# BenjSta/bernoulli-var-speech-codec

Measured on AMD Instinct MI355X. Metric: audio-seconds coded per wall-second (encode+decode), 22.05 kHz @ 3 kbit/s, higher is better.
Workload: dtype f32; 1 GPU; BASELINE configs[1]: batch 64 x 5 s utterances per GPU, config_varBitRate @ 3000 bit/s (35 bits/frame), full encode -> BigVGAN decode; one batch at a time on one stream; frames_per_utterance=430, weights=seeded synthetic (checkpoints are LFS pointers), gather=none, streams=1

## Files before the change

bernoulli-var-speech-codec_amd/csrc/bvc_internal.h:

```cpp
#pragma once
#include <hip/hip_runtime.h>
#include <stdint.h>
#include <string>
#include <vector>

#include "../../include/bvcodec.h"

namespace bvc {

void set_error(const char *fmt, ...);

#define BVC_HIP_TRY(expr)                                                              \
    do {                                                                               \
        hipError_t e_ = (expr);                                                        \
        if (e_ != hipSuccess) {                                                        \
            bvc::set_error("%s failed: %s (%s:%d)", #expr, hipGetErrorString(e_), __FILE__, __LINE__); \
            return BVC_EHIP;                                                           \
        }                                                                              \
    } while (0)

enum ProbeKind { PK_NONE = 0, PK_LINEAR = 1, PK_GRU = 2, PK_CONV = 3, PK_BATCHED = 4, PK_STFT = 5, PK_POST = 6 };
struct ProbeScope {
    hipStream_t s; int slot;
    ProbeScope(int kind, hipStream_t stream);
// ... 101 lines not shown
    int wnb;
    int pad_;
};
struct FlowArgs {
    FlowLin enc0h, enc1, enc2, pz0, pz1, pz2, dec0h, dec0z, dec1, dec2, dec3, px0, px1, px2;
    const float *w_hh, *w_ihx, *w_ihz;
    const float *b_ih, *b_hh;
    int hb, zb, xb;
    float *flow; unsigned slot_bytes;
    int B, MT, NTG;
    long long T;
    const float *part0;
    const float *part_gru;
    float *codes, *prob; const float *bits; float *all_h; float *mel;
    const float *mean, *stdv;
    int var_bit;
    unsigned *status; unsigned spin_limit;
    unsigned long long *probe;
    int probe_nodes, probe_first;
    int probe_wg, probe_wave;
    int dbg_hot_w;
    int MG;
    int dbg_withhold;
    FlowLin pxc;
    float *keep;
};
int flow_kernels_init();
int flow_perh(int h_dim);
int launch_flow(const FlowArgs &a, FlowArgs *d_args, int perh, bool encode, bool fill, hipStream_t s, bool args_resident = false);
int launch_flow_prepare(const FlowArgs &a, FlowArgs *d_args, unsigned *flow, long long n_flow, long long n_h0, const float *d_h0, int B, int H,
                        hipStream_t s);
int launch_flow_census(unsigned *ctr, int grid, unsigned spin_limit, hipStream_t s);
int launch_fill_u32(unsigned *p, unsigned v, long long n, hipStream_t s);

struct FrontendTables {
    const float *window;
    const float2 *tw1;
    const float2 *tw2;
    const float2 *tws;
    const int   *mel_start;
    const int   *mel_len;
    const int   *mel_off;
    const float *mel_w;
    int num_mels;
    int kmax;
};
int launch_stft_logmel(const FrontendTables &t, const float *wav, int B, long long L, long long T,
                       int pad_left, float scale, float *mel, hipStream_t s, const long long *lens = nullptr);
__host__ __device__ inline long long ragged_frames(long long len, long long L, int pad_left) {
    len = len < 0 ? 0 : (len > L ? L : len);
    const long long pr = 1024 - 256 - pad_left;
    if (len <= pad_left || len <= pr) return 0;
    return (len + pad_left + pr - 1024) / 256 + 1;
}
int launch_ragged_bits(float *bits, const float *d_bits, float dflt, const long long *lens, int B, long long L, long long T,
                       int pad_left, hipStream_t s);
int launch_ragged_mask(float *codes, const long long *lens, int B, long long L, long long T, int z, int pad_left, hipStream_t s);

int launch_resample_poly(const float *x, int B, long long Lin, const double *h, int ntaps, int up, int down,
                         long long n_pre_remove, float *y, long long n_out, hipStream_t s);
int launch_peak_normalize(float *x, int B, long long L, hipStream_t s);
int launch_pack_codes(const float *codes, long long frames, int z, int nbits, unsigned char *out, hipStream_t s);
int launch_unpack_codes(const unsigned char *in, long long frames, int z, int nbits, float *codes, hipStream_t s);

struct ConvLayer {
    int cin;
    int cout;
    int ntiles;
    int ks;
    int dil;
    const float *wp;
    const float *wp4;
    const float *wp2;
    const float *bias;
    const float *act_a;
    const float *act_ib;
};
enum ConvEpi { CE_STORE = 0, CE_RES = 1, CE_RES_ACC = 2, CE_RES_ACC_DIV = 3 };
#ifdef BVC_PHASE_PROBE
int phase_probe_read(unsigned long long *out, int reset);
#endif
struct ConvWindow { long long in_bs, out_bs, row_begin, t_origin; };
int conv_kernels_init();
enum : unsigned { AMPK_C8 = 1u, AMPK_C16 = 2u, AMPK_ALL = 3u };
unsigned amp_kernels_default();
int launch_snakebeta_test(const float *x, long long n, float a, float ib, float *y, hipStream_t s);
int launch_conv_mfma(const ConvLayer &c, const float *in, long long Lin, float *out, long long Lout,
                     int B, int epi, const float *res, const float *acc, float divisor, hipStream_t s,
                     const ConvWindow *win = nullptr, const long long *row_lim = nullptr);
int launch_amp_pair(const ConvLayer &c1, const ConvLayer &c2, const float *x, long long L, float *out, int B, int epi,
                    const float *acc, float divisor, hipStream_t s, const ConvWindow *win = nullptr, unsigned kernels = AMPK_ALL);
int launch_conv_post(const float *in, long long Lin, int C, int ks, const float *w, const float *bias,
                     const float *act_a, const float *act_ib, float div, float *wav, long long n_out,
                     int B, hipStream_t s, const ConvWindow *win = nullptr, const long long *n_rows = nullptr);
int launch_ragged_limits(long long *lim, const long long *frames, const long long *lengths, int B, long long T, long long n_max,
                         int n_up, const int *up_rates, hipStream_t s);

}
```

bernoulli-var-speech-codec_amd/csrc/bvcodec_abi.hip:

```cpp
#include <algorithm>
#include <atomic>
#include <cmath>
#include <cstdarg>
#include <cstdio>
#include <cstdlib>
#include <cstring>
#include <list>
#include <map>
#include <memory>
#include <mutex>

#include "bvc_internal.h"

namespace bvc {

static thread_local char g_err[512] = "";

void set_error(const char *fmt, ...) {
    va_list ap;
    va_start(ap, fmt);
    vsnprintf(g_err, sizeof(g_err), fmt, ap);
    va_end(ap);
}

// ... 1963 lines not shown
    hipStream_t s = (hipStream_t)stream;
    const int B = st->B;
    sc_append_kernel<<<dim3((unsigned)((st->hop + 255) / 256), B), 256, 0, s>>>(st->d_state, st->d_in, st->hop, st->sbuf, st->cap);
    if (st->first) {
        sc_reflect_left_kernel<<<dim3(B), 256, 0, s>>>(st->sbuf, st->cap, c.pad_left);
        st->first = false;
    }
    BVC_HIP_TRY(hipGetLastError());
    const int fill = st->fill + st->hop;
    const int k = fill >= c.n_fft ? (fill - c.n_fft) / c.hop + 1 : 0;
    if (k > st->kmax) { set_error("bvc_stream_codec_tick: internal frame count %d", k); return BVC_EINVAL; }
    int rc = BVC_OK;
    if (k > 0) {
        const int parity = st->voc->parity;
        const bool tick_flow = st->tick_flow && flow_chains_static(st->m, B) != 0;
        const bool warm = !tick_flow && !st->voc->slide && st->use_graph && s != nullptr && st->frames >= STREAM_WARM_FRAMES;
        g_stream_tick = true; g_tick_flow = tick_flow;
        if (!warm) {
            rc = stream_tick_body(st, k, s);
        } else {
            hipGraphExec_t &ge = st->graph[k][parity];
            if (!ge) {
                hipGraph_t graph = nullptr;
                const int vp = st->voc->parity; const int64_t vf = st->voc->frames;
                g_capturing = true;
                hipError_t e = hipStreamBeginCapture(s, hipStreamCaptureModeThreadLocal);
                if (e == hipSuccess) rc = stream_tick_body(st, k, s);
                hipError_t e2 = (e == hipSuccess) ? hipStreamEndCapture(s, &graph) : e;
                g_capturing = false;
                st->voc->parity = vp; st->voc->frames = vf;
                if (!rc && (e2 != hipSuccess || !graph)) { set_error("bvc_stream_codec_tick: hipGraph capture failed: %s", hipGetErrorString(e2)); rc = BVC_EHIP; }
                if (!rc && hipGraphInstantiate(&ge, graph, nullptr, nullptr, 0) != hipSuccess) { set_error("bvc_stream_codec_tick: hipGraphInstantiate failed"); rc = BVC_EHIP; }
                if (graph) (void)hipGraphDestroy(graph);
            }
            if (!rc) {
                if (hipGraphLaunch(ge, s) != hipSuccess) { set_error("bvc_stream_codec_tick: hipGraphLaunch failed"); rc = BVC_EHIP; }
                st->voc->parity ^= 1; st->voc->frames += k;
            }
        }
        g_stream_tick = false; g_tick_flow = false;
        if (rc) return rc;
    }
    sc_advance_kernel<<<1, 64, 0, s>>>(st->d_state, st->hop - c.hop * k);
    BVC_HIP_TRY(hipGetLastError());
    st->fill = fill - c.hop * k;
    st->frames += k;
    st->ticks += 1;
    if (n_frames) *n_frames = k;
    return BVC_OK;
}

int bvc_model_set_option(bvc_model *m, const char *name, int32_t value) {
    if (!m || !name) { set_error("bvc_model_set_option: null argument"); return BVC_EINVAL; }
    if (strcmp(name, "recurrence") == 0) {
        if (value < 0 || value > 2) { set_error("bvc_model_set_option: recurrence must be 0 (persistent), 1 (layers) or 2 (auto)"); return BVC_EINVAL; }
        m->recurrence = value;
        return BVC_OK;
    }
    if (strcmp(name, "flow_spin_limit") == 0) {
        if (value < 1) { set_error("bvc_model_set_option: flow_spin_limit must be positive"); return BVC_EINVAL; }
        m->flow_spin_limit = (unsigned)value;
        return BVC_OK;
    }
    if (strcmp(name, "flow_debug_withhold") == 0) {
        m->flow_debug_withhold = value != 0;
        return BVC_OK;
    }
    if (strcmp(name, "decode_fold") == 0) {
        m->decode_fold = value != 0;
        return BVC_OK;
    }
    if (strcmp(name, "encode_fold") == 0) {
        m->encode_fold = value != 0;
        return BVC_OK;
    }
    if (strcmp(name, "flow_debug_nofill") == 0) {
        m->flow_debug_nofill = value != 0;
        return BVC_OK;
    }
    if (strcmp(name, "vocoder_c16_kernel") == 0) {
        m->amp_kernels = value ? (m->amp_kernels | AMPK_C16) : (m->amp_kernels & ~AMPK_C16);
        return BVC_OK;
    }
    if (strcmp(name, "vocoder_full_tiles") == 0) {
        m->amp_kernels = value ? (m->amp_kernels | AMPK_C8) : (m->amp_kernels & ~AMPK_C8);
        return BVC_OK;
    }
    set_error("bvc_model_set_option: unknown option '%s'", name);
    return BVC_EINVAL;
}

int bvc_flow_fence(void *stream) {
    hipStream_t s = (hipStream_t)stream;
    hipStreamCaptureStatus cs = hipStreamCaptureStatusNone;
    BVC_HIP_TRY(hipStreamIsCapturing(s, &cs));
    if (cs != hipStreamCaptureStatusNone) { set_error("bvc_flow_fence: not while the stream is being captured"); return BVC_EINVAL; }
    int dev = 0;
    BVC_HIP_TRY(hipGetDevice(&dev));
    dev &= 15;
    std::lock_guard<std::mutex> lk(g_flow_mu);
    FlowFence &f = g_fence[dev][g_fence_n[dev]++ % FLOW_FENCES];
    if (!f.ev) BVC_HIP_TRY(hipEventCreateWithFlags(&f.ev, hipEventDisableTiming));
    if (f.pending) BVC_HIP_TRY(hipStreamWaitEvent(s, f.ev, 0));
    BVC_HIP_TRY(hipEventRecord(f.ev, s));
    f.pending = true;
    return BVC_OK;
}

int bvc_model_get_option(const bvc_model *m, const char *name, int32_t *value) {
    if (!m || !name || !value) { set_error("bvc_model_get_option: null argument"); return BVC_EINVAL; }
    if (strcmp(name, "recurrence") == 0) { *value = m->recurrence; return BVC_OK; }
    if (strcmp(name, "decode_fold") == 0) { *value = m->decode_fold; return BVC_OK; }
    if (strcmp(name, "encode_fold") == 0) { *value = m->encode_fold; return BVC_OK; }
    if (strcmp(name, "flow_resident") == 0) { *value = m->flow_resident ? 1 : 0; return BVC_OK; }
    if (strcmp(name, "flow_supported") == 0) { *value = m->flow_perh > 0 ? 1 : 0; return BVC_OK; }
    if (strcmp(name, "compute_units") == 0) { *value = m->cu_count; return BVC_OK; }
    set_error("bvc_model_get_option: unknown option '%s'", name);
    return BVC_EINVAL;
}

int bvc_model_status(const bvc_model *m, uint32_t *code) {
    if (!m) { set_error("null model"); return BVC_EINVAL; }
    unsigned v = 0;
    if (m->h_status) {
        BVC_HIP_TRY(hipDeviceSynchronize());
        v = *m->h_status;
        if (v) { *m->h_status = 0u; m->census_due = true; }
    }
    if (code) *code = v;
    if (v) {
        set_error("a persistent recurrence kernel gave up waiting (frame %u, layer %u): its results are invalid",
                  (v & 0x7FFFFFFFu) >> 4, (v & 15u));
        return BVC_ETIMEOUT;
    }
    return BVC_OK;
}

int bvc_model_poll_status(const bvc_model *m, uint32_t *code) {
    if (!m) { set_error("null model"); return BVC_EINVAL; }
    unsigned v = 0;
    if (m->h_status) {
        v = *m->h_status;
        if (v) { *m->h_status = 0u; m->census_due = true; }
    }
    if (code) *code = v;
    if (v) {
        set_error("a persistent recurrence kernel gave up waiting (frame %u, layer %u): the results of the call that has just been "
                  "synchronised are invalid.  All its workgroups must be resident together - is another process using this GPU?",
                  (v & 0x7FFFFFFFu) >> 4, (v & 15u));
        return BVC_ETIMEOUT;
    }
    return BVC_OK;
}

int bvc_probe_begin(int32_t kind, int32_t sample_every, int32_t max_samples) {
    if (kind <= PK_NONE || kind > PK_POST || sample_every < 1 || max_samples < 1) {
        set_error("bvc_probe_begin: bad arguments");
        return BVC_EINVAL;
    }
    while ((int)g_probe.ev.size() < 2 * max_samples) {
        hipEvent_t e;
        BVC_HIP_TRY(hipEventCreate(&e));
        g_probe.ev.push_back(e);
    }
    g_probe.kind = kind; g_probe.every = sample_every; g_probe.counter = 0; g_probe.used = 0;
    return BVC_OK;
// ... 159 lines not shown
```

bernoulli-var-speech-codec_amd/csrc/k_vocoder.hip:

```cpp
#include <cstdlib>
#include <type_traits>

#include "bvc_internal.h"

namespace bvc {

typedef float f32x4 __attribute__((ext_vector_type(4)));

__device__ __forceinline__ void divide_if(bool div, f32x4 &v, float d) {
    if (div) {
        asm volatile("" ::: "memory");
#pragma unroll
        for (int e = 0; e < 4; ++e) v[e] = v[e] / d;
    }
}

__device__ __forceinline__ unsigned div_tpb(unsigned bid, unsigned tpb_magic) { return __umulhi(bid, tpb_magic); }
static inline unsigned tpb_magic_of(unsigned d) { return d <= 1u ? 0xFFFFFFFFu : (unsigned)(0x100000000ull / d) + 1u; }

__device__ __forceinline__ __amdgpu_buffer_rsrc_t rows_rsrc(const float *base, long long L, int C) {
    return __builtin_amdgcn_make_buffer_rsrc(const_cast<float *>(base), 0, (int)(L * C * 4), 0x00020000);
}
__device__ __forceinline__ f32x4 rows_load4(__amdgpu_buffer_rsrc_t rs, int row, int C, int c0) {
    return __builtin_bit_cast(f32x4, __builtin_amdgcn_raw_buffer_load_b128(rs, (row * C + c0) * 4, 0, 0));
// ... 367 lines not shown
            const float hi1 = __int_as_float(__builtin_amdgcn_update_dpp(0, __float_as_int(a3), 0x118, 0xf, 0xf, false));
            const float v0 = r < 8 ? a0 : hi0, v1 = r < 8 ? a1 : hi1;
            const int row = mbase + i * 16 + g * 4 + e0;
            const f32x2 s2 = snakebeta2((f32x2){v0 + bias, v1 + bias}, splat2(aa), splat2(bb));
            t2[row * S + col] = row >= zrow ? s2[0] : 0.0f;
            t2[(row + 1) * S + col] = row + 1 >= zrow ? s2[1] : 0.0f;
        }
    } else {
        auto s2_tile = [&](auto edge_c) {
            constexpr bool EDGE = decltype(edge_c)::value;
#pragma unroll
            for (int n = 0; n < NTL; ++n) {
                const int col = (nt0 + n) * 16 + r;
                if (col < C) {
                    const float bias = a.b1[col], aa = a.a2[col], bb = a.ib2[col];
#pragma unroll
                    for (int i = 0; i < MT; ++i)
#pragma unroll
                        for (int e = 0; e < 4; e += 2) {
                            const int row = mbase + i * 16 + g * 4 + e;
                            const f32x2 u2 = (f32x2){acc[i][n][e] + bias, acc[i][n][e + 1] + bias};
                            const f32x2 s2 = snakebeta2(u2, splat2(aa), splat2(bb));
                            t2[row * S + col] = (!EDGE || row >= zrow) ? s2[0] : 0.0f;
                            t2[(row + 1) * S + col] = (!EDGE || row + 1 >= zrow) ? s2[1] : 0.0f;
                        }
                }
            }
        };
        if (zrow > 0) s2_tile(std::true_type());
        else          s2_tile(std::false_type());
    }
    __syncthreads();
    PHASE(2);

    const long long ob = (long long)b * a.bs + t0 * C;
    constexpr int NLD3 = (TR * C4 + 255) / 256;
    const long long rows_left = a.L - t0;
    const int nvalid4 = (int)(rows_left < TT ? rows_left : TT) * C4;
    f32x4 resq[NLD3], accq[NLD3];
    const bool with_acc = a.epi >= CE_RES_ACC;
#pragma unroll
    for (int i = 0; i < NLD3; ++i) {
        const int idx = tid + i * 256;
        const int idc = idx < nvalid4 ? idx : 0;
        resq[i] = reinterpret_cast<const f32x4 *>(a.x + ob)[idc];
        accq[i] = with_acc ? reinterpret_cast<const f32x4 *>(a.acc + ob)[idc] : (f32x4){0.f, 0.f, 0.f, 0.f};
    }
    PHASE(3);
    conv(t2, 1, a.w2);
    PHASE(4);
    if (ALIAS) __syncthreads();
#pragma unroll
    for (int n = 0; n < NTL; ++n) {
        const int col = (nt0 + n) * 16 + r;
        if (col >= C) continue;
        const float bias = a.b2[col];
#pragma unroll
        for (int i = 0; i < MT; ++i)
#pragma unroll
            for (int e = 0; e < 4; ++e) t1[(mbase + i * 16 + g * 4 + e) * S + col] = acc[i][n][e] + bias;
    }
    __syncthreads();
#pragma unroll
    for (int i = 0; i < NLD3; ++i) {
        const int idx = tid + i * 256;
        if (idx >= nvalid4) continue;
        const int row = idx / C4, c4 = idx - row * C4;
        const float2 lo = *reinterpret_cast<const float2 *>(t1 + row * S + c4 * 4);
        const float2 hi = *reinterpret_cast<const float2 *>(t1 + row * S + c4 * 4 + 2);
        f32x4 v = (f32x4){lo.x, lo.y, hi.x, hi.y};
#pragma unroll
        for (int e = 0; e < 4; ++e) {
            float o = v[e] + resq[i][e];
            if (a.epi >= CE_RES_ACC) o = accq[i][e] + o;
            v[e] = o;
        }
        divide_if(a.epi == CE_RES_ACC_DIV, v, a.divisor);
        reinterpret_cast<f32x4 *>(a.out + ob)[idx] = v;
    }
    PHASE(5);
}

unsigned amp_kernels_default() {
    return (getenv("BVC_NO_AMP8") == nullptr ? AMPK_C8 : 0u) | (getenv("BVC_NO_AMP16") == nullptr ? AMPK_C16 : 0u);
}

template <int D>
__device__ __forceinline__ int pair_row(int m) { return (m / D) * (2 * D) + m % D; }
template <int D>
__device__ __forceinline__ int row_pos(int rho, int H) {
    const int blk = rho / (2 * D), w = rho - blk * (2 * D);
    return w >= D ? H + blk * D + (w - D) : blk * D + w;
}
template <int KS, int D, int MT2>
struct Amp8Geom {
    static constexpr int NP = 4 * MT2 * 16;
    static constexpr int NPE = (NP / D) * D;
    static constexpr int TR1 = 2 * NPE;
    static constexpr int TR = 2 * NP;
    static constexpr int TT = TR1 - (KS - 1);
    static constexpr int HALO1 = (KS - 1) * D;
    static constexpr int ROWS1 = TR1 + HALO1;
    static constexpr int H1 = NP + ((KS + 1) / 2) * D;
    static constexpr int H2 = NP + (KS + 1) / 2;
    static constexpr int S = 10;
    static constexpr int LDS_ROWS = 2 * H1 > TR ? 2 * H1 : TR;
    static constexpr size_t LDS_BYTES = (size_t)LDS_ROWS * S * sizeof(float);
};

template <int KS, int D, int MT2, int OCC>
__global__ __launch_bounds__(256, OCC) void amp_pair8_kernel(AmpArgs a) {
    extern __shared__ __attribute__((aligned(16))) float lds[];
    using G = Amp8Geom<KS, D, MT2>;
    constexpr int C = 8, S = G::S, NP = G::NP, NPE = G::NPE, TR = G::TR, TT = G::TT, H1 = G::H1, H2 = G::H2;
    constexpr int NLD = (G::ROWS1 * 2 + 255) / 256;
    const int tid = threadIdx.x, lane = tid & 63;
    const int wave = __builtin_amdgcn_readfirstlane(tid >> 6);
    const int r = lane & 15, g = lane >> 4;
    const unsigned per = (a.ntile + 7u) >> 3, nli = gridDim.x >> 3;
    const unsigned xcd = blockIdx.x & 7u;
    unsigned li = blockIdx.x >> 3;
    const unsigned run_end = (xcd + 1u) * per < a.ntile ? (xcd + 1u) * per : a.ntile;
    if (xcd * per + li >= run_end) return;

    float w1reg[KS + 1][2], w2reg[KS + 1][2];
#pragma unroll
    for (int k = 0; k <= KS; ++k)
#pragma unroll
        for (int q = 0; q < 2; ++q) {
            w1reg[k][q] = a.w1[(k * 2 + q) * 64 + lane];
            w2reg[k][q] = a.w2[(k * 2 + q) * 64 + lane];
        }
    const f32x4 aa1 = *reinterpret_cast<const f32x4 *>(a.a1 + (tid & 1) * 4);
    const f32x4 bb1 = *reinterpret_cast<const f32x4 *>(a.ib1 + (tid & 1) * 4);
    const int p = g >> 1, co0 = (g & 1) * 4;
    const f32x4 bias1 = *reinterpret_cast<const f32x4 *>(a.b1 + co0), aa2 = *reinterpret_cast<const f32x4 *>(a.a2 + co0);
    const f32x4 bb2 = *reinterpret_cast<const f32x4 *>(a.ib2 + co0), bias2 = *reinterpret_cast<const f32x4 *>(a.b2 + co0);

    auto tile_origin = [&](unsigned bid, int &b, long long &t0) {
        b = a.tiles_per_batch == 1 ? (int)bid : (int)div_tpb(bid, a.tpb_magic);
        t0 = a.row_begin + (long long)(bid - (unsigned)b * (unsigned)a.tiles_per_batch) * TT;
    };
    auto load_rows = [&](unsigned bid, f32x4 (&v)[NLD]) {
        int b; long long t0;
        tile_origin(bid, b, t0);
        const __amdgpu_buffer_rsrc_t rs = rows_rsrc(a.x + (long long)b * a.bs, a.L, C);
        const int tfirst = (int)(t0 - (KS - 1) - G::HALO1);
#pragma unroll
        for (int i = 0; i < NLD; ++i) {
            const int idx = tid + i * 256;
            v[i] = rows_load4(rs, tfirst + (idx >> 1), C, (idx & 1) * 4);
        }
    };

    const int mbase = wave * MT2 * 16;
    f32x4 acc[MT2];
    auto conv = [&](auto dd, int H, const float (&wreg)[KS + 1][2]) {
        constexpr int DD = decltype(dd)::value;
        const float *arow = lds + (mbase + r) * S + g;
#pragma unroll
        for (int i = 0; i < MT2; ++i) acc[i] = (f32x4){0.f, 0.f, 0.f, 0.f};
#pragma unroll
        for (int k = 0; k <= KS; ++k) {
            const int pos = (k >> 1) * DD + (k & 1) * H;
#pragma unroll
            for (int q = 0; q < 2; ++q) {
                float av[MT2];
// ... 291 lines not shown
        f32x4 resq[MT], accq[MT];
#pragma unroll
        for (int i = 0; i < MT; ++i) {
            const int row = mbase + i * 16 + r;
            const bool ok = row < nvalid;
            resq[i] = ok ? *reinterpret_cast<const f32x4 *>(a.x + ob + row * C + g * 4) : (f32x4){0.f, 0.f, 0.f, 0.f};
            accq[i] = (ok && a.epi >= CE_RES_ACC) ? *reinterpret_cast<const f32x4 *>(a.acc + ob + row * C + g * 4) : (f32x4){0.f, 0.f, 0.f, 0.f};
        }
        conv(std::integral_constant<int, 1>(), t2, w2reg);
#pragma unroll
        for (int i = 0; i < MT; ++i) {
            const int row = mbase + i * 16 + r;
            if (row >= nvalid) continue;
            f32x4 o4 = acc[i] + bias2;
#pragma unroll
            for (int e = 0; e < 4; ++e) {
                float o = o4[e] + resq[i][e];
                if (a.epi >= CE_RES_ACC) o = accq[i][e] + o;
                o4[e] = o;
            }
            divide_if(a.epi == CE_RES_ACC_DIV, o4, a.divisor);
            *reinterpret_cast<f32x4 *>(a.out + ob + row * C + g * 4) = o4;
        }
        if (!more) break;
    }
}

template <int KS, int D, int MT, int OCC>
static int amp16_slots() {
    static int slots = 0;
    if (!slots) {
        int per_cu = 0, dev = 0, cus = 0;
        if (hipGetDevice(&dev) != hipSuccess || hipDeviceGetAttribute(&cus, hipDeviceAttributeMultiprocessorCount, dev) != hipSuccess ||
            hipOccupancyMaxActiveBlocksPerMultiprocessor(&per_cu, reinterpret_cast<const void *>(amp_pair16_kernel<KS, D, MT, OCC>), 256,
                                                         Amp16Geom<KS, D, MT>::LDS_BYTES) != hipSuccess) {
            set_error("amp_pair16: occupancy query failed");
            return -1;
        }
        slots = (per_cu > 0 ? per_cu : 1) * cus;
    }
    return slots;
}
template <int KS, int D, int MT, int OCC>
static int launch_amp16_t(AmpArgs a, int B, hipStream_t s) {
    using G = Amp16Geom<KS, D, MT>;
    a.tiles_per_batch = (int)((a.L - a.row_begin + G::TT - 1) / G::TT);
    if (a.tiles_per_batch <= 0) return BVC_OK;
    a.tpb_magic = tpb_magic_of((unsigned)a.tiles_per_batch);
    if ((unsigned long long)a.tiles_per_batch * a.tiles_per_batch * (unsigned long long)B >= 0x100000000ull) { set_error("vocoder: tile count beyond the reciprocal's range"); return BVC_EINVAL; }
    const int slots = amp16_slots<KS, D, MT, OCC>();
    if (slots <= 0) return BVC_EHIP;
    ProbeScope probe(PK_CONV, s);
    const unsigned ntile = (unsigned)(a.tiles_per_batch * (long long)B);
    a.ntile = ntile;
    const unsigned grid = ntile < (unsigned)slots ? ((ntile + 7u) & ~7u) : ((unsigned)slots & ~7u);
    hipLaunchKernelGGL((amp_pair16_kernel<KS, D, MT, OCC>), dim3(grid), dim3(256), G::LDS_BYTES, s, a);
    BVC_HIP_TRY(hipGetLastError());
    return BVC_OK;
}
template <int KS, int MT> struct Amp16Occ { static constexpr int V = MT >= 4 ? 2 : (KS == 3 ? 4 : KS == 7 ? 3 : 2); };
template <int MT>
static int launch_amp16(AmpArgs a, int B, hipStream_t s) {
    switch (a.ks * 8 + a.dil) {
        case 3 * 8 + 1:  return launch_amp16_t<3, 1, MT, Amp16Occ<3, MT>::V>(a, B, s);
        case 3 * 8 + 3:  return launch_amp16_t<3, 3, MT, Amp16Occ<3, MT>::V>(a, B, s);
        case 3 * 8 + 5:  return launch_amp16_t<3, 5, MT, Amp16Occ<3, MT>::V>(a, B, s);
        case 7 * 8 + 1:  return launch_amp16_t<7, 1, MT, Amp16Occ<7, MT>::V>(a, B, s);
        case 7 * 8 + 3:  return launch_amp16_t<7, 3, MT, Amp16Occ<7, MT>::V>(a, B, s);
        case 7 * 8 + 5:  return launch_amp16_t<7, 5, MT, Amp16Occ<7, MT>::V>(a, B, s);
        case 11 * 8 + 1: return launch_amp16_t<11, 1, (MT > 4 ? 4 : MT), Amp16Occ<11, MT>::V>(a, B, s);
        case 11 * 8 + 3: return launch_amp16_t<11, 3, (MT > 4 ? 4 : MT), Amp16Occ<11, MT>::V>(a, B, s);
        case 11 * 8 + 5: return launch_amp16_t<11, 5, (MT > 4 ? 4 : MT), Amp16Occ<11, MT>::V>(a, B, s);
        default: return -1;
    }
}
template <int MT>
static bool amp16_slots_all() {
    return amp16_slots<3, 1, MT, Amp16Occ<3, MT>::V>() > 0 && amp16_slots<3, 3, MT, Amp16Occ<3, MT>::V>() > 0 && amp16_slots<3, 5, MT, Amp16Occ<3, MT>::V>() > 0 &&
           amp16_slots<7, 1, MT, Amp16Occ<7, MT>::V>() > 0 && amp16_slots<7, 3, MT, Amp16Occ<7, MT>::V>() > 0 && amp16_slots<7, 5, MT, Amp16Occ<7, MT>::V>() > 0 &&
           amp16_slots<11, 1, (MT > 4 ? 4 : MT), Amp16Occ<11, MT>::V>() > 0 && amp16_slots<11, 3, (MT > 4 ? 4 : MT), Amp16Occ<11, MT>::V>() > 0 &&
           amp16_slots<11, 5, (MT > 4 ? 4 : MT), Amp16Occ<11, MT>::V>() > 0;
}

template <int C, int MT, int OCC, bool ALIAS, int CS = 1>
static int launch_amp_t(AmpArgs a, int B, hipStream_t s) {
    constexpr int TR = (4 / CS) * MT * 16;
    const int TT = TR - (a.ks - 1);
    a.tiles_per_batch = (int)((a.L - a.row_begin + TT - 1) / TT);
    if (a.tiles_per_batch <= 0) return BVC_OK;
    a.tpb_magic = tpb_magic_of((unsigned)a.tiles_per_batch);
    if ((unsigned long long)a.tiles_per_batch * a.tiles_per_batch * (unsigned long long)B >= 0x100000000ull) { set_error("vocoder: tile count beyond the reciprocal's range"); return BVC_EINVAL; }
    const size_t lds = (size_t)((TR + (a.ks - 1) * a.dil) + (ALIAS ? 0 : TR + (a.ks - 1))) * (C + 2) * sizeof(float);
    if (lds > 160 * 1024 || TT <= 0) { set_error("amp_pair tile needs %zu B of LDS", lds); return BVC_EINVAL; }
    ProbeScope probe(PK_CONV, s);
    const unsigned ntile = (unsigned)(a.tiles_per_batch * (long long)B);
    a.ntile = ntile;
    {
        static bool attr = false;
        if (!attr) { BVC_HIP_TRY(hipFuncSetAttribute(reinterpret_cast<const void *>(amp_pair_kernel<C, MT, OCC, ALIAS, CS>), hipFuncAttributeMaxDynamicSharedMemorySize, 160 * 1024)); attr = true; }
    }
    hipLaunchKernelGGL((amp_pair_kernel<C, MT, OCC, ALIAS, CS>), dim3((ntile + 7u) & ~7u), dim3(256), lds, s, a);
    BVC_HIP_TRY(hipGetLastError());
    return BVC_OK;
}

int launch_amp_pair(const ConvLayer &c1, const ConvLayer &c2, const float *x, long long L, float *out, int B, int epi,
                    const float *acc, float divisor, hipStream_t s, const ConvWindow *win, unsigned kernels) {
    if (B <= 0 || L <= 0) return BVC_OK;
    if (c1.cin != c1.cout || c2.cin != c1.cin || c2.ks != c1.ks || c2.dil != 1 || !c1.act_a || !c2.act_a) {
        set_error("amp_pair: unsupported layer pair");
        return BVC_EINVAL;
    }
    AmpArgs a;
    a.x = x; a.out = out; a.acc = acc; a.L = L;
    a.w1 = c1.wp; a.b1 = c1.bias; a.a1 = c1.act_a; a.ib1 = c1.act_ib;
    a.w2 = c2.wp; a.b2 = c2.bias; a.a2 = c2.act_a; a.ib2 = c2.act_ib;
    if (c1.cin >= 32) {
        if (!c1.wp4 || !c2.wp4) { set_error("amp_pair: layer pair without the 16-byte weight packing"); return BVC_EINVAL; }
        a.w1 = c1.wp4; a.w2 = c2.wp4;
    }
    a.divisor = divisor; a.epi = epi; a.ks = c1.ks; a.dil = c1.dil; a.tiles_per_batch = 0;
    a.bs = win ? win->in_bs : L * c1.cin;
    a.row_begin = win ? win->row_begin : 0;
    a.t_origin = win ? win->t_origin : 0;
    const long long new_rows = L - a.row_begin;
    if (win && c1.cin == 64 && new_rows <= 32 - (c1.ks - 1)) return launch_amp_t<64, 2, 2, true, 4>(a, B, s);
    if (win && c1.cin == 64 && new_rows <= 2 * (64 - (c1.ks - 1))) return launch_amp_t<64, 1, 2, true>(a, B, s);
    static const int s32 = getenv("BVC_AMP32S") ? atoi(getenv("BVC_AMP32S")) : 3;
    if (win && c1.cin == 32 && new_rows <= s32 * (64 - (c1.ks - 1))) return launch_amp_t<32, 1, 3, true>(a, B, s);
    if (c1.cin == 8 && c1.wp2 && c2.wp2 && (kernels & AMPK_C8)) {
        AmpArgs a8 = a;
        a8.w1 = c1.wp2; a8.w2 = c2.wp2;
        const int rc8 = (win && new_rows <= 128) ? launch_amp8<1, 4>(a8, B, s) : launch_amp8<2, 2>(a8, B, s);
        if (rc8 != -1) return rc8;
    }
    switch (c1.cin) {
        case 64: {
            static const bool rows = getenv("BVC_AMP64") && atoi(getenv("BVC_AMP64")) == 0;
            if (rows) return launch_amp_t<64, 2, 2, true>(a, B, s);
            return launch_amp_t<64, 8, 2, true, 4>(a, B, s);
        }
        case 32: return launch_amp_t<32, 4, 3, true>(a, B, s);
        case 16: {
            if ((kernels & AMPK_C16) && !win) {
                const int rc16 = launch_amp16<4>(a, B, s);
                if (rc16 != -1) return rc16;
            }
            return launch_amp_t<16, 2, 4, false>(a, B, s);
        }
        case 8:  return launch_amp_t<8, 4, 4, true>(a, B, s);
        default: set_error("amp_pair: unsupported channel count %d", c1.cin); return BVC_EINVAL;
    }
}

template <int CIN, int NTW, int MT, bool NSPLIT = false>
static int launch_one(const ConvArgs &a, int B, hipStream_t s) {
    constexpr int TT = (NSPLIT ? 1 : 4) * MT * 16;
    ConvArgs k = a;
    k.tiles_per_batch = (int)((a.Lout - a.row_begin + TT - 1) / TT);
    if (k.tiles_per_batch <= 0) return BVC_OK;
    const size_t lds = (size_t)(TT + (a.ks - 1) * a.dil) * (CIN + 2) * sizeof(float);
    if (lds > 160 * 1024) { set_error("conv tile needs %zu B of LDS", lds); return BVC_EINVAL; }
    constexpr int NPW = NTW * (NSPLIT ? 4 : 1);
    dim3 grid((unsigned)(k.tiles_per_batch * (long long)B), (unsigned)((a.ntiles + NPW - 1) / NPW));
    auto kern = conv_mfma_kernel<CIN, NTW, MT, NSPLIT>;
    ProbeScope probe(PK_CONV, s);
    hipLaunchKernelGGL(kern, grid, dim3(256), lds, s, k);
    BVC_HIP_TRY(hipGetLastError());
    return BVC_OK;
}

template <int CIN, int NTW, int MT, bool NSPLIT = false>
static int allow_big_lds() {
    BVC_HIP_TRY(hipFuncSetAttribute(reinterpret_cast<const void *>(conv_mfma_kernel<CIN, NTW, MT, NSPLIT>),
                                    hipFuncAttributeMaxDynamicSharedMemorySize, 160 * 1024));
    return BVC_OK;
}

__global__ void snakebeta_test_kernel(const float *__restrict__ x, long long n, float a, float ib, float *__restrict__ y) {
    for (long long i = ((long long)blockIdx.x * blockDim.x + threadIdx.x) * 2; i < n; i += (long long)gridDim.x * blockDim.x * 2) {
        if (i + 1 < n && !(i & 2)) {
            const f32x2 v = snakebeta2((f32x2){x[i], x[i + 1]}, splat2(a), splat2(ib));
            y[i] = v[0];
            y[i + 1] = v[1];
        } else {
            y[i] = snakebeta(x[i], a, ib);
            if (i + 1 < n) y[i + 1] = snakebeta(x[i + 1], a, ib);
        }
    }
}

int launch_snakebeta_test(const float *x, long long n, float a, float ib, float *y, hipStream_t s) {
    if (n <= 0) return BVC_OK;
    hipLaunchKernelGGL(snakebeta_test_kernel, dim3(256), dim3(256), 0, s, x, n, a, ib, y);
    BVC_HIP_TRY(hipGetLastError());
    return BVC_OK;
}

int conv_kernels_init() {
    int rc;
    if (!amp8_slots_all<1, 4>() || !amp8_slots_all<2, 2>()) return BVC_EHIP;
    if (!amp16_slots_all<4>()) return BVC_EHIP;
    if ((rc = allow_big_lds<128, 4, 2>())) return rc;
    if ((rc = allow_big_lds<80, 4, 2>())) return rc;
    if ((rc = allow_big_lds<64, 4, 2>())) return rc;
    if ((rc = allow_big_lds<32, 2, 4>())) return rc;
    if ((rc = allow_big_lds<16, 1, 4>())) return rc;
    if ((rc = allow_big_lds<8, 1, 4>())) return rc;
    return BVC_OK;
}

int launch_conv_mfma(const ConvLayer &c, const float *in, long long Lin, float *out, long long Lout, int B,
                     int epi, const float *res, const float *acc, float divisor, hipStream_t s, const ConvWindow *win,
                     const long long *row_lim) {
    if (B <= 0 || Lout <= 0) return BVC_OK;
    if (c.cout % 4) { set_error("conv_mfma: %d output columns (the epilogue stores 16-byte granules)", c.cout); return BVC_EINVAL; }
    ConvArgs a;
    a.in = in; a.Lin = Lin; a.out = out; a.Lout = Lout; a.res = res; a.acc = acc;
    a.in_bs = win ? win->in_bs : Lin * c.cin;
    a.out_bs = win ? win->out_bs : Lout * c.cout;
    a.row_begin = win ? win->row_begin : 0;
    a.wp = c.wp; a.bias = c.bias; a.act_a = c.act_a; a.act_ib = c.act_ib;
    a.divisor = divisor; a.epi = epi; a.ks = c.ks; a.dil = c.dil; a.cout = c.cout; a.ntiles = c.ntiles;
    a.tiles_per_batch = 0;
    a.row_lim = row_lim;
    if (win && Lout - a.row_begin <= 16) {
        switch (c.cin) {
            case 128: return launch_one<128, 4, 1, true>(a, B, s);
            case 80:  return launch_one<80, 2, 1, true>(a, B, s);
            case 64:  return launch_one<64, 4, 1, true>(a, B, s);
            default: break;
        }
    }
    switch (c.cin) {
        case 128: return launch_one<128, 4, 2>(a, B, s);
        case 80:  return launch_one<80, 4, 2>(a, B, s);
        case 64:  return launch_one<64, 4, 2>(a, B, s);
        case 32:  return launch_one<32, 2, 4>(a, B, s);
        case 16:  return launch_one<16, 1, 4>(a, B, s);
        case 8:   return launch_one<8, 1, 4>(a, B, s);
        default:
            set_error("conv_mfma: unsupported input channel count %d", c.cin);
            return BVC_EINVAL;
    }
}

template <int C>
__global__ __launch_bounds__(256) void conv_post_kernel(const float *__restrict__ in, long long Lin, int ks,
                                                        const float *__restrict__ w, const float *__restrict__ bias,
                                                        const float *__restrict__ act_a,
                                                        const float *__restrict__ act_ib, float div,
                                                        float *__restrict__ wav, long long n_out,
                                                        int tiles_per_batch, long long in_bs, long long row_begin,
                                                        const long long *__restrict__ n_rows) {
    extern __shared__ __attribute__((aligned(16))) float tile[];
    const int tid = threadIdx.x;
    const int b = blockIdx.x / tiles_per_batch;
    const long long t0 = row_begin + (long long)(blockIdx.x % tiles_per_batch) * 256;
    const int halo = ks - 1;
    const float *inb = in + (long long)b * in_bs;
    for (int idx = tid; idx < (256 + halo) * C; idx += 256) {
        const int row = idx / C, c = idx - row * C;
        const long long tg = t0 - halo + row;
        float v = 0.0f;
        if (tg >= 0 && tg < Lin) v = snakebeta(inb[tg * C + c], act_a[c], act_ib[c]);
        tile[idx] = v;
    }
    __syncthreads();
    const long long t = t0 + tid - row_begin;
    if (t >= n_out) return;
    if (n_rows && t >= n_rows[b]) { wav[(long long)b * n_out + t] = 0.0f; return; }
    float acc = 0.0f;
    for (int j = 0; j < ks; ++j)
#pragma unroll
        for (int c = 0; c < C; ++c) acc = fmaf(w[c * ks + j], tile[(tid + j) * C + c], acc);
    wav[(long long)b * n_out + t] = tanhf(acc + bias[0]) / div;
}

int launch_conv_post(const float *in, long long Lin, int C, int ks, const float *w, const float *bias,
                     const float *act_a, const float *act_ib, float div, float *wav, long long n_out, int B,
                     hipStream_t s, const ConvWindow *win, const long long *n_rows) {
    if (B <= 0 || n_out <= 0) return BVC_OK;
    if (C != 8) { set_error("conv_post: unsupported channel count %d", C); return BVC_EINVAL; }
    const int tiles = (int)((n_out + 255) / 256);
    const size_t lds = (size_t)(256 + ks - 1) * C * sizeof(float);
// ... 43 lines not shown
```

Measured before the change: 6987 audio-seconds/s.

## Add persistent run-based fused AMP pair kernel for 32/64-channel vocoder blocks

Adds a persistent kernel for the 32- and 64-channel resblock conv pairs (snake, conv, snake, conv, residual). Each block walks a contiguous run of rows along time and carries the conv halos in LDS between tiles, so halo rows are no longer recomputed or reloaded per tile. It also prefetches the next tile's input and double-buffers the weight chunks. The grid is sized to the occupancy slots and the kernel is enabled by default for non-windowed calls. The cost is less parallelism per batch item, since runs are serial along time, plus a more complex schedule and extra synchronisation.

```diff
diff --git a/bernoulli-var-speech-codec_amd/csrc/bvc_internal.h b/bernoulli-var-speech-codec_amd/csrc/bvc_internal.h
--- a/bernoulli-var-speech-codec_amd/csrc/bvc_internal.h
+++ b/bernoulli-var-speech-codec_amd/csrc/bvc_internal.h
@@ -207,7 +207,7 @@
 #endif
 struct ConvWindow { long long in_bs, out_bs, row_begin, t_origin; };
 int conv_kernels_init();
-enum : unsigned { AMPK_C8 = 1u, AMPK_C16 = 2u, AMPK_ALL = 3u };
+enum : unsigned { AMPK_C8 = 1u, AMPK_C16 = 2u, AMPK_C32 = 4u, AMPK_C64 = 8u, AMPK_ALL = 15u };
 unsigned amp_kernels_default();
 int launch_snakebeta_test(const float *x, long long n, float a, float ib, float *y, hipStream_t s);
 int launch_conv_mfma(const ConvLayer &c, const float *in, long long Lin, float *out, long long Lout,
diff --git a/bernoulli-var-speech-codec_amd/csrc/bvcodec_abi.hip b/bernoulli-var-speech-codec_amd/csrc/bvcodec_abi.hip
--- a/bernoulli-var-speech-codec_amd/csrc/bvcodec_abi.hip
+++ b/bernoulli-var-speech-codec_amd/csrc/bvcodec_abi.hip
@@ -2069,6 +2069,14 @@
         m->amp_kernels = value ? (m->amp_kernels | AMPK_C16) : (m->amp_kernels & ~AMPK_C16);
         return BVC_OK;
     }
+    if (strcmp(name, "vocoder_c32_kernel") == 0) {
+        m->amp_kernels = value ? (m->amp_kernels | AMPK_C32) : (m->amp_kernels & ~AMPK_C32);
+        return BVC_OK;
+    }
+    if (strcmp(name, "vocoder_c64_kernel") == 0) {
+        m->amp_kernels = value ? (m->amp_kernels | AMPK_C64) : (m->amp_kernels & ~AMPK_C64);
+        return BVC_OK;
+    }
     if (strcmp(name, "vocoder_full_tiles") == 0) {
         m->amp_kernels = value ? (m->amp_kernels | AMPK_C8) : (m->amp_kernels & ~AMPK_C8);
         return BVC_OK;
diff --git a/bernoulli-var-speech-codec_amd/csrc/k_vocoder.hip b/bernoulli-var-speech-codec_amd/csrc/k_vocoder.hip
--- a/bernoulli-var-speech-codec_amd/csrc/k_vocoder.hip
+++ b/bernoulli-var-speech-codec_amd/csrc/k_vocoder.hip
@@ -473,7 +473,7 @@
 }
 
 unsigned amp_kernels_default() {
-    return (getenv("BVC_NO_AMP8") == nullptr ? AMPK_C8 : 0u) | (getenv("BVC_NO_AMP16") == nullptr ? AMPK_C16 : 0u);
+    return (getenv("BVC_NO_AMP8") == nullptr ? AMPK_C8 : 0u) | (getenv("BVC_NO_AMP16") == nullptr ? AMPK_C16 : 0u) | AMPK_C32 | AMPK_C64;
 }
 
 template <int D>
@@ -931,6 +931,276 @@
            amp16_slots<11, 5, (MT > 4 ? 4 : MT), Amp16Occ<11, MT>::V>() > 0;
 }
 
+template <int C, int KS, int D, int MT, int CS>
+struct AmpRunGeom {
+    static constexpr int S = C + 2;
+    static constexpr int TR = (4 / CS) * MT * 16;
+    static constexpr int HALO1 = (KS - 1) * D;
+    static constexpr int ROWS1 = HALO1 + TR;
+    static constexpr int ROWS2 = (KS - 1) + TR;
+    static constexpr size_t LDS_BYTES = (size_t)(ROWS1 + ROWS2) * S * sizeof(float);
+    static_assert(TR >= HALO1, "a carry's source and destination rows must not overlap");
+};
+
+template <int C, int KS, int D, int MT, int CS, int OCC>
+__global__ __launch_bounds__(256, OCC) void amp_run_kernel(AmpArgs a) {
+    extern __shared__ __attribute__((aligned(16))) float lds[];
+    using G = AmpRunGeom<C, KS, D, MT, CS>;
+    constexpr int S = G::S, TR = G::TR, HALO1 = G::HALO1, C4 = C / 4, NT = C / 16, NTL = NT / CS;
+    constexpr int CGU = C4 < 16 / NTL ? C4 : 16 / NTL;
+    static_assert(NT % CS == 0 && CGU % 4 == 0 && C4 % CGU == 0 && 256 % C4 == 0 && (TR * C4) % 256 == 0, "unsupported shape");
+    constexpr int G4 = CGU / 4, CPT = C4 / CGU, NCH = KS * CPT;
+    constexpr int NLD = TR * C4 / 256;
+    float *t1 = lds, *t2 = lds + G::ROWS1 * S;
+    const int tid = threadIdx.x, lane = tid & 63;
+    const int wave = __builtin_amdgcn_readfirstlane(tid >> 6);
+    const int r = lane & 15, g = lane >> 4;
+    const int mbase = (wave / CS) * MT * 16, nt0 = (wave % CS) * NTL;
+    const int c4 = tid % C4;
+    const f32x4 aa1 = *reinterpret_cast<const f32x4 *>(a.a1 + c4 * 4), bb1 = *reinterpret_cast<const f32x4 *>(a.ib1 + c4 * 4);
+
+    auto park_s1 = [&](const f32x4 &v, int row) {
+        f32x4 o;
+#pragma unroll
+        for (int e = 0; e < 4; e += 2) {
+            const f32x2 o2 = snakebeta2((f32x2){v[e], v[e + 1]}, (f32x2){aa1[e], aa1[e + 1]}, (f32x2){bb1[e], bb1[e + 1]});
+            o[e] = o2[0]; o[e + 1] = o2[1];
+        }
+        float2 *dst = reinterpret_cast<float2 *>(t1 + row * S + c4 * 4);
+        dst[0] = make_float2(o[0], o[1]);
+        dst[1] = make_float2(o[2], o[3]);
+    };
+
+    f32x4 acc[MT][NTL];
+    auto conv = [&](const float *tile, auto dd, const float *wp, auto &&hook) {
+        constexpr int DD = decltype(dd)::value;
+        static_assert(NCH >= 2, "the first two chunks are peeled");
+#pragma unroll
+        for (int i = 0; i < MT; ++i)
+#pragma unroll
+            for (int n = 0; n < NTL; ++n) acc[i][n] = (f32x4){0.f, 0.f, 0.f, 0.f};
+        f32x4 bcur[G4][NTL], bnxt[G4][NTL];
+        auto loadb = [&](f32x4 (&dstb)[G4][NTL], int q) {
+            const f32x4 *wq = reinterpret_cast<const f32x4 *>(wp) + (long long)q * G4 * NT * 64 + lane;
+#pragma unroll
+            for (int u = 0; u < G4; ++u)
+#pragma unroll
+                for (int n = 0; n < NTL; ++n) dstb[u][n] = wq[(u * NT + nt0 + n) * 64];
+        };
+        auto compute = [&](const f32x4 (&bw)[G4][NTL], int q) {
+            const int j = q / CPT, cg0 = (q - j * CPT) * CGU;
+            const float *brow = tile + (mbase + r + j * DD) * S + g;
+#pragma unroll
+            for (int u = 0; u < CGU; ++u) {
+                float bv[MT];
+#pragma unroll
+                for (int i = 0; i < MT; ++i) bv[i] = brow[i * 16 * S + (cg0 + u) * 4];
+#pragma unroll
+                for (int i = 0; i < MT; ++i)
+#pragma unroll
+                    for (int n = 0; n < NTL; ++n)
+                        acc[i][n] = __builtin_amdgcn_mfma_f32_16x16x4f32(bw[u >> 2][n][u & 3], bv[i], acc[i][n], 0, 0, 0);
+            }
+        };
+        loadb(bcur, 0);
+        loadb(bnxt, 1);
+        hook();
+        __builtin_amdgcn_sched_barrier(0);
+        compute(bcur, 0);
+        __builtin_amdgcn_sched_barrier(0);
+        loadb(bcur, 2 < NCH ? 2 : NCH - 1);
+        __builtin_amdgcn_sched_barrier(0);
+        compute(bnxt, 1);
+        __builtin_amdgcn_sched_barrier(0);
+        int q = 2;
+#pragma unroll 1
+        for (; q + 1 < NCH; q += 2) {
+            loadb(bnxt, q + 1);
+            __builtin_amdgcn_sched_barrier(0);
+            compute(bcur, q);
+            __builtin_amdgcn_sched_barrier(0);
+            loadb(bcur, q + 2 < NCH ? q + 2 : NCH - 1);
+            __builtin_amdgcn_sched_barrier(0);
+            compute(bnxt, q + 1);
+            __builtin_amdgcn_sched_barrier(0);
+        }
+        if (q < NCH) compute(bcur, q);
+    };
+
+    const int R = a.tiles_per_batch;
+    const bool with_acc = a.epi >= CE_RES_ACC;
+#pragma unroll 1
+    for (unsigned run = blockIdx.x; run < a.ntile; run += gridDim.x) {
+        const int b = (int)(run / (unsigned)R), kr = (int)(run - (unsigned)b * (unsigned)R);
+        const long long r0 = a.L * kr / R, r1 = a.L * (kr + 1) / R;
+        const long long p0 = r0 - (KS - 1);
+        const int ntl = (int)((r1 - p0 + TR - 1) / TR);
+        const __amdgpu_buffer_rsrc_t rs = rows_rsrc(a.x + (long long)b * a.bs, a.L, C);
+        f32x4 v[NLD];
+#pragma unroll
+        for (int i = 0; i < NLD; ++i) v[i] = rows_load4(rs, (int)p0 + (tid + i * 256) / C4, C, c4 * 4);
+        __syncthreads();
+        for (int idx = tid; idx < HALO1 * C4; idx += 256) park_s1(rows_load4(rs, (int)(p0 - HALO1) + idx / C4, C, c4 * 4), idx / C4);
+        for (int idx = tid; idx < (KS - 1) * S; idx += 256) t2[idx] = 0.0f;
+#pragma unroll 1
+        for (int k = 0; k < ntl; ++k) {
+            const long long tb = p0 + (long long)k * TR;
+            if (k > 0) {
+                __syncthreads();
+                for (int idx = tid; idx < (KS - 1) * C; idx += 256) {
+                    const int row = idx / C, c = idx - row * C;
+                    t2[row * S + c] = t2[(TR + row) * S + c];
+                }
+            }
+#pragma unroll
+            for (int i = 0; i < NLD; ++i) park_s1(v[i], HALO1 + (tid + i * 256) / C4);
+            __syncthreads();
+
+            conv(t1, std::integral_constant<int, D>(), a.w1, [&] {
+#pragma unroll
+                for (int i = 0; i < NLD; ++i) v[i] = rows_load4(rs, (int)(tb + TR) + (tid + i * 256) / C4, C, c4 * 4);
+            });
+            __syncthreads();
+            {
+                const long long zr64 = -tb;
+                const int zrow = zr64 <= 0 ? 0 : (zr64 > TR ? TR : (int)zr64);
+                auto s2_tile = [&](auto edge_c) {
+                    constexpr bool EDGE = decltype(edge_c)::value;
+#pragma unroll
+                    for (int n = 0; n < NTL; ++n) {
+                        const int col = (nt0 + n) * 16 + g * 4;
+                        const f32x4 bias = *reinterpret_cast<const f32x4 *>(a.b1 + col);
+                        const f32x4 aa = *reinterpret_cast<const f32x4 *>(a.a2 + col), bb = *reinterpret_cast<const f32x4 *>(a.ib2 + col);
+#pragma unroll
+                        for (int i = 0; i < MT; ++i) {
+                            const int m = mbase + i * 16 + r;
+                            const f32x4 u4 = acc[i][n] + bias;
+                            const f32x2 s01 = snakebeta2((f32x2){u4[0], u4[1]}, (f32x2){aa[0], aa[1]}, (f32x2){bb[0], bb[1]});
+                            const f32x2 s23 = snakebeta2((f32x2){u4[2], u4[3]}, (f32x2){aa[2], aa[3]}, (f32x2){bb[2], bb[3]});
+                            const bool keep = !EDGE || m >= zrow;
+                            float2 *dst = reinterpret_cast<float2 *>(t2 + (KS - 1 + m) * S + col);
+                            dst[0] = keep ? make_float2(s01[0], s01[1]) : make_float2(0.f, 0.f);
+                            dst[1] = keep ? make_float2(s23[0], s23[1]) : make_float2(0.f, 0.f);
+                        }
+                    }
+                };
+                if (zrow > 0) s2_tile(std::true_type());
+                else          s2_tile(std::false_type());
+            }
+            for (int idx = tid; idx < HALO1 * C4; idx += 256) {
+                const int row = idx / C4;
+                const float2 *src = reinterpret_cast<const float2 *>(t1 + (TR + row) * S + c4 * 4);
+                float2 *dst = reinterpret_cast<float2 *>(t1 + row * S + c4 * 4);
+                const float2 lo = src[0], hi = src[1];
+                dst[0] = lo;
+                dst[1] = hi;
+            }
+            __syncthreads();
+
+            f32x4 resq[MT][NTL], accq[MT][NTL];
+            conv(t2, std::integral_constant<int, 1>(), a.w2, [&] {
+                const __amdgpu_buffer_rsrc_t ra = rows_rsrc(a.acc + (long long)b * a.bs, a.L, C);
+#pragma unroll
+                for (int i = 0; i < MT; ++i)
+#pragma unroll
+                    for (int n = 0; n < NTL; ++n) {
+                        const int row = (int)tb + mbase + i * 16 + r, col = (nt0 + n) * 16 + g * 4;
+                        resq[i][n] = rows_load4(rs, row, C, col);
+                        accq[i][n] = with_acc ? rows_load4(ra, row, C, col) : (f32x4){0.f, 0.f, 0.f, 0.f};
+                    }
+            });
+            float *oo = a.out + (long long)b * a.bs;
+#pragma unroll
+            for (int n = 0; n < NTL; ++n) {
+                const int col = (nt0 + n) * 16 + g * 4;
+                const f32x4 bias = *reinterpret_cast<const f32x4 *>(a.b2 + col);
+#pragma unroll
+                for (int i = 0; i < MT; ++i) {
+                    const long long row = tb + mbase + i * 16 + r;
+                    if (row < r0 || row >= r1) continue;
+                    f32x4 o4 = acc[i][n] + bias;
+#pragma unroll
+                    for (int e = 0; e < 4; ++e) {
+                        float o = o4[e] + resq[i][n][e];
+                        if (with_acc) o = accq[i][n][e] + o;
+                        o4[e] = o;
+                    }
+                    divide_if(a.epi == CE_RES_ACC_DIV, o4, a.divisor);
+                    *reinterpret_cast<f32x4 *>(oo + row * C + col) = o4;
+                }
+            }
+        }
+    }
+}
+
+template <int C, int KS, int D, int MT, int CS, int OCC>
+static int amprun_slots() {
+    static int slots = 0;
+    if (!slots) {
+        const void *f = reinterpret_cast<const void *>(amp_run_kernel<C, KS, D, MT, CS, OCC>);
+        const size_t lds = AmpRunGeom<C, KS, D, MT, CS>::LDS_BYTES;
+        int per_cu = 0, dev = 0, cus = 0;
+        const bool ok = hipGetDevice(&dev) == hipSuccess && hipDeviceGetAttribute(&cus, hipDeviceAttributeMultiprocessorCount, dev) == hipSuccess &&
+                        hipFuncSetAttribute(f, hipFuncAttributeMaxDynamicSharedMemorySize, (int)lds) == hipSuccess &&
+                        hipOccupancyMaxActiveBlocksPerMultiprocessor(&per_cu, f, 256, lds) == hipSuccess && per_cu > 0;
+        if (!ok) (void)hipGetLastError();
+        slots = ok ? per_cu * cus : -1;
+    }
+    return slots;
+}
+template <int C, int KS, int D, int MT, int CS, int OCC>
+static int launch_amprun_t(AmpArgs a, int B, hipStream_t s) {
+    using G = AmpRunGeom<C, KS, D, MT, CS>;
+    if ((a.L + 2 * G::TR + G::HALO1) * C * 4 >= 0x80000000ll) return -1;
+    const int slots = amprun_slots<C, KS, D, MT, CS, OCC>();
+    if (slots <= 0) return -1;
+    long long runs = slots / B;
+    const long long most = (a.L + G::TR - 1) / G::TR;
+    if (runs > most) runs = most;
+    if (runs < 1) runs = 1;
+    a.tiles_per_batch = (int)runs;
+    a.ntile = (unsigned)(runs * B);
+    const unsigned grid = a.ntile < (unsigned)slots ? a.ntile : (unsigned)slots;
+    ProbeScope probe(PK_CONV, s);
+    hipLaunchKernelGGL((amp_run_kernel<C, KS, D, MT, CS, OCC>), dim3(grid), dim3(256), G::LDS_BYTES, s, a);
+    BVC_HIP_TRY(hipGetLastError());
+    return BVC_OK;
+}
+template <int C> struct AmpRunShape;
+template <> struct AmpRunShape<32> { static constexpr int MT = 4, CS = 1, OCC = 2; };
+template <> struct AmpRunShape<64> { static constexpr int MT = 4, CS = 4, OCC = 2; };
+template <int C, int KS, int D>
+static int launch_amprun_s(AmpArgs a, int B, hipStream_t s) {
+    using P = AmpRunShape<C>;
+    return launch_amprun_t<C, KS, D, P::MT, P::CS, P::OCC>(a, B, s);
+}
+template <int C, int KS, int D>
+static bool amprun_ready() {
+    using P = AmpRunShape<C>;
+    return amprun_slots<C, KS, D, P::MT, P::CS, P::OCC>() > 0;
+}
+template <int C>
+static int launch_amprun(AmpArgs a, int B, hipStream_t s) {
+    switch (a.ks * 8 + a.dil) {
+        case 3 * 8 + 1:  return launch_amprun_s<C, 3, 1>(a, B, s);
+        case 3 * 8 + 3:  return launch_amprun_s<C, 3, 3>(a, B, s);
+        case 3 * 8 + 5:  return launch_amprun_s<C, 3, 5>(a, B, s);
+        case 7 * 8 + 1:  return launch_amprun_s<C, 7, 1>(a, B, s);
+        case 7 * 8 + 3:  return launch_amprun_s<C, 7, 3>(a, B, s);
+        case 7 * 8 + 5:  return launch_amprun_s<C, 7, 5>(a, B, s);
+        case 11 * 8 + 1: return launch_amprun_s<C, 11, 1>(a, B, s);
+        case 11 * 8 + 3: return launch_amprun_s<C, 11, 3>(a, B, s);
+        case 11 * 8 + 5: return launch_amprun_s<C, 11, 5>(a, B, s);
+        default: return -1;
+    }
+}
+template <int C>
+static void amprun_init() {
+    (void)amprun_ready<C, 3, 1>(); (void)amprun_ready<C, 3, 3>(); (void)amprun_ready<C, 3, 5>();
+    (void)amprun_ready<C, 7, 1>(); (void)amprun_ready<C, 7, 3>(); (void)amprun_ready<C, 7, 5>();
+    (void)amprun_ready<C, 11, 1>(); (void)amprun_ready<C, 11, 3>(); (void)amprun_ready<C, 11, 5>();
+}
+
 template <int C, int MT, int OCC, bool ALIAS, int CS = 1>
 static int launch_amp_t(AmpArgs a, int B, hipStream_t s) {
     constexpr int TR = (4 / CS) * MT * 16;
@@ -985,11 +1255,21 @@
     }
     switch (c1.cin) {
         case 64: {
+            if ((kernels & AMPK_C64) && !win) {
+                const int rc = launch_amprun<64>(a, B, s);
+                if (rc != -1) return rc;
+            }
             static const bool rows = getenv("BVC_AMP64") && atoi(getenv("BVC_AMP64")) == 0;
             if (rows) return launch_amp_t<64, 2, 2, true>(a, B, s);
             return launch_amp_t<64, 8, 2, true, 4>(a, B, s);
         }
-        case 32: return launch_amp_t<32, 4, 3, true>(a, B, s);
+        case 32: {
+            if ((kernels & AMPK_C32) && !win) {
+                const int rc = launch_amprun<32>(a, B, s);
+                if (rc != -1) return rc;
+            }
+            return launch_amp_t<32, 4, 3, true>(a, B, s);
+        }
         case 16: {
             if ((kernels & AMPK_C16) && !win) {
                 const int rc16 = launch_amp16<4>(a, B, s);
@@ -1050,6 +1330,8 @@
     int rc;
     if (!amp8_slots_all<1, 4>() || !amp8_slots_all<2, 2>()) return BVC_EHIP;
     if (!amp16_slots_all<4>()) return BVC_EHIP;
+    amprun_init<32>();
+    amprun_init<64>();
     if ((rc = allow_big_lds<128, 4, 2>())) return rc;
     if ((rc = allow_big_lds<80, 4, 2>())) return rc;
     if ((rc = allow_big_lds<64, 4, 2>())) return rc;
```

Result: no change. 7017 audio-seconds/s (median of 6 runs) (+0.4%).
